# cisco/openh264

Measured on AMD Instinct MI355X. Metric: 1080p frames/sec/GPU at QP=24 CBP; encoder_binary_comparison SHA1 pass, higher is better.
Workload: dtype u8

## Files before the change

### openh264_amd/csrc/kernels/inter_mb.h

```cpp
#pragma once
#include "frame_kernels.h"
#include "../common/gom_rc.h"


#if defined(WH_EMU)
#include <stdio.h>
static long g_wh_win_stat[40];
static void wh_win_stat_dump() {
  if (!getenv ("WELSHIP_WIN_STATS")) return;
  fprintf (stderr, "welship mb stat: skip %ld bg/static %ld intra %ld p16x16 %ld p16x8 %ld p8x16 %ld p8x8 %ld renamed-skip %ld | searches 16x16 %ld 16x8/8x16 %ld 8x8 %ld, diamond steps %ld %ld %ld | refinements %ld %ld %ld | skip tests %ld with transform %ld\n",
           g_wh_win_stat[8], g_wh_win_stat[9], g_wh_win_stat[10], g_wh_win_stat[11], g_wh_win_stat[12], g_wh_win_stat[13], g_wh_win_stat[14], g_wh_win_stat[15], g_wh_win_stat[16], g_wh_win_stat[17], g_wh_win_stat[18],
           g_wh_win_stat[19], g_wh_win_stat[20], g_wh_win_stat[21], g_wh_win_stat[22], g_wh_win_stat[23], g_wh_win_stat[24], g_wh_win_stat[25], g_wh_win_stat[26]);
  fprintf (stderr, "welship window stat: P macroblocks %ld, reloads %ld, adopted %ld, first loads %ld, mid-walk reloads %ld, chroma predictions inside the window %ld / from the picture %ld\n", g_wh_win_stat[0], g_wh_win_stat[1], g_wh_win_stat[2], g_wh_win_stat[3], g_wh_win_stat[4], g_wh_win_stat[5], g_wh_win_stat[6]);
}
struct WhWinStatInit { WhWinStatInit() { atexit (wh_win_stat_dump); } };
static WhWinStatInit g_wh_win_stat_init;
#define WH_STAT_WIN(i) (++g_wh_win_stat[i])
#define WH_STAT_BLK(base, bw, bh) (++g_wh_win_stat[(base) + ((bw) == 16 && (bh) == 16 ? 0 : (bw) == 8 && (bh) == 8 ? 2 : 1)])
#else
#define WH_STAT_WIN(i) ((void)0)
#define WH_STAT_BLK(base, bw, bh) ((void)0)
#endif

#define WH_REF_NOT_AVAIL (-2)
#define WH_REF_NOT_IN_LIST (-1)
#define WH_WIN_STRIDE 80
#ifndef WH_WIN_ROWS
#define WH_WIN_ROWS 38
#endif
#define WH_WIN_MARGIN_X 19
#ifndef WH_WIN_MARGIN_Y
#define WH_WIN_MARGIN_Y 11
#endif
#ifndef WH_WIN_START
// ... 339 lines not shown
}

WH_FN void wh_slot_geom (int slot, int* bx, int* by, int* bw, int* bh) {
  if (slot == 0) { *bx = 0; *by = 0; *bw = 16; *bh = 16; }
  else if (slot < WH_SLOT_16x8) { const int i = slot - WH_SLOT_8x8; *bx = (i & 1) * 8; *by = (i >> 1) * 8; *bw = 8; *bh = 8; }
  else if (slot < WH_SLOT_8x16) { const int i = slot - WH_SLOT_16x8; *bx = 0; *by = i * 8; *bw = 16; *bh = 8; }
  else { const int i = slot - WH_SLOT_8x16; *bx = i * 8; *by = 0; *bw = 8; *bh = 16; }
}
WH_FN void wh_slot_pred (const WhMvCache& K, int slot, int* mx, int* my) {
  if (slot == 0) wh_pred_mv (K, 0, 0, 4, 0, mx, my);
  else if (slot < WH_SLOT_16x8) { const int i = slot - WH_SLOT_8x8; wh_pred_mv (K, (i & 1) * 2, (i >> 1) * 2, 2, 0, mx, my); }
  else if (slot < WH_SLOT_8x16) wh_pred_16x8 (K, slot - WH_SLOT_16x8, 0, mx, my);
  else wh_pred_8x16 (K, slot - WH_SLOT_8x16, 0, mx, my);
}

typedef struct WhMe {
  int bx, by, bw, bh;
  int mvpx, mvpy;
  int sad_pred;
  int mvx, mvy;
  int sad_cost, satd_cost;
  int satd_raw;
} WhMe;

typedef struct WhMeCtx {
  int mbx, mby, lambda, use_satd;
  int minx, miny, maxx, maxy;
} WhMeCtx;

WH_FN int wh_cand_sad (const WhInterLds& S, const WhSeqParams& P, const WhPicJob& J, const WhWin& W, const WhMeCtx& C, const WhMe& me, int imx, int imy) {
  const int px = C.mbx * 16 + me.bx + imx, py = C.mby * 16 + me.by + imy;
  if (wh_win_covers (W, px, py, px + me.bw + 3, py + me.bh))
    return wh_sad_win (S, W, me.bx, me.by, me.bw, me.bh, (py - W.y0) * WH_WIN_STRIDE + px - W.x0);
  return wh_sad_global (S, P, J, me.bx, me.by, me.bw, me.bh, px, py);
}

typedef struct WhSccMe {
  const WH_G WhSccJob* job;
  int method;
  uint32_t thr;
  int dir_on, dmx, dmy;
  uint32_t chain;
  uint32_t fme_down;
} WhSccMe;

WH_FN void wh_line_search (const WhInterLds& S, const WhSeqParams& P, const WhPicJob& J, WhWin& W, const WhMeCtx& C, const WhMe& me, bool vertical, int* best, int* bmx, int* bmy) {
  const int lo = vertical ? C.miny : C.minx, hi = vertical ? C.maxy : C.maxx;
  const int px = C.mbx * 16 + me.bx, py = C.mby * 16 + me.by;
  const WH_G uint8_t* ref = (const WH_G uint8_t*)J.ref[0];
// ... 70 lines not shown
    }
    if (stop) break;
  }
  *best = b;
}

WH_FN void wh_me_satd (WhInterLds& S, const WhWin& W, const WhMeCtx& C, WhMe& me, int bmx, int bmy) {
  const int wo = (C.mby * 16 + me.by + bmy - W.y0) * WH_WIN_STRIDE + C.mbx * 16 + me.bx + bmx - W.x0;
  const int nq = (me.bw >> 2) * (me.bh >> 2) * 4;
  WV_SATD_ROWS (me.satd_raw, lane, lane < nq,
                wh_enc4 (S, me.bx + (lane < nq ? wh_tl_col (lane, me.bw) : 0), me.by + (lane < nq ? wh_tl_row (lane, me.bw) : 0)),
                wh_ld4u (W.b->win, wo + (lane < nq ? wh_tl_row (lane, me.bw) * WH_WIN_STRIDE + wh_tl_col (lane, me.bw) : 0)));
  me.satd_cost = me.satd_raw + wh_mvd_cost (C.lambda, me.mvx - me.mvpx, me.mvy - me.mvpy);
}

WH_FN void wh_motion_search (WhInterLds& S, const WhSeqParams& P, const WhPicJob& J, WhWin& W, const WhMeCtx& C, WhMe& me, const WvLaneArr& mvcl, int n_mvc, WhSccMe* Z = nullptr) {
  int bmx = wh_clip3 ((2 + me.mvpx) >> 2, C.minx, C.maxx), bmy = wh_clip3 ((2 + me.mvpy) >> 2, C.miny, C.maxy);
  int best = wh_cand_sad (S, P, J, W, C, me, bmx, bmy) + wh_mvd_cost (C.lambda, bmx * 4 - me.mvpx, bmy * 4 - me.mvpy);
  for (int i = 0; i < n_mvc; ++i) {
    const int cand = WV_LGET (mvcl, i);
    const int cx = wh_clip3 ((2 + wh_mvx (cand)) >> 2, C.minx, C.maxx), cy = wh_clip3 ((2 + wh_mvy (cand)) >> 2, C.miny, C.maxy);
    if (cx != bmx || cy != bmy) {
      const int c = wh_cand_sad (S, P, J, W, C, me, cx, cy) + wh_mvd_cost (C.lambda, cx * 4 - me.mvpx, cy * 4 - me.mvpy);
      if (c < best) { best = c; bmx = cx; bmy = cy; }
    }
  }
  if (Z && Z->dir_on && (Z->dmx | Z->dmy) && Z->dmx >= C.minx && Z->dmx < C.maxx && Z->dmy >= C.miny && Z->dmy < C.maxy) {
    const int c = wh_cand_sad (S, P, J, W, C, me, Z->dmx, Z->dmy) + wh_mvd_cost (C.lambda, Z->dmx * 4 - me.mvpx, Z->dmy * 4 - me.mvpy);
    if ((uint32_t)c < Z->chain) { best = c; bmx = Z->dmx; bmy = Z->dmy; WH_STAT (WH_ST_DIR_TAKEN); }
  }
  const bool diamond = !(best < me.sad_pred);
  WH_STAT_BLK (16, me.bw, me.bh);
  const int bpx = C.mbx * 16 + me.bx, bpy = C.mby * 16 + me.by;
  if (diamond || C.use_satd) wh_win_need (S, P, J, W, bpx + bmx, bpy + bmy, me.bw, me.bh, diamond ? WH_WIN_START : 0);
  if (diamond) {
    int dx = bmx * 4 - me.mvpx, dy = bmy * 4 - me.mvpy;
    int wo = (bpy + bmy - W.y0) * WH_WIN_STRIDE + bpx + bmx - W.x0;
    const int n = (me.bw * me.bh) >> 2;
    int budget = wh_win_room (W, bpx + bmx, bpy + bmy, me.bw, me.bh);
    for (int it = 0; it < 16; ++it) {
      const int cmx = (dx + me.mvpx) >> 2, cmy = (dy + me.mvpy) >> 2;
      if (!(cmx >= C.minx && cmx < C.maxx && cmy >= C.miny && cmy < C.maxy)) break;
      if (it >= budget) {
        if (wh_win_room (W, bpx + cmx, bpy + cmy, me.bw, me.bh) < 1) {
          WH_STAT_WIN (4);
          wh_win_need (S, P, J, W, bpx + cmx, bpy + cmy, me.bw, me.bh, WH_WIN_START);
          wo = (bpy + cmy - W.y0) * WH_WIN_STRIDE + bpx + cmx - W.x0;
        }
        budget = it + wh_max (1, wh_win_room (W, bpx + cmx, bpy + cmy, me.bw, me.bh));
      }
#if defined(WH_EMU)
      if (wh_win_room (W, bpx + cmx, bpy + cmy, me.bw, me.bh) < 1 || wo != (bpy + cmy - W.y0) * WH_WIN_STRIDE + bpx + cmx - W.x0) { fprintf (stderr, "emu: diamond step outside the search window\n"); abort(); }
#endif
      WH_STAT_BLK (19, me.bw, me.bh);
      int pud, plr;
      WV_SUM2 (pud, plr, lane,
               (lane < n ? ([&] () { const int r = wh_sl_row (lane, me.bw), c = wh_sl_col (lane, me.bw);
                                     const uint32_t e = wh_enc4 (S, me.bx + c, me.by + r); const int o = wo + r * WH_WIN_STRIDE + c;
                                     return wh_sad4 (e, wh_ld4u (W.b->win, o - WH_WIN_STRIDE)) | (wh_sad4 (e, wh_ld4u (W.b->win, o + WH_WIN_STRIDE)) << 16); }) () : 0),
               (lane < n ? ([&] () { const int r = wh_sl_row (lane, me.bw), c = wh_sl_col (lane, me.bw);
                                     const uint32_t e = wh_enc4 (S, me.bx + c, me.by + r); const int o = wo + r * WH_WIN_STRIDE + c;
                                     return wh_sad4 (e, wh_ld4u (W.b->win, o - 1)) | (wh_sad4 (e, wh_ld4u (W.b->win, o + 1)) << 16); }) () : 0));
      const int c0 = (pud & 0xffff) + wh_mvd_cost (C.lambda, dx, dy - 4);
      const int c1 = (int) ((unsigned)pud >> 16) + wh_mvd_cost (C.lambda, dx, dy + 4);
      const int c2 = (plr & 0xffff) + wh_mvd_cost (C.lambda, dx - 4, dy);
      const int c3 = (int) ((unsigned)plr >> 16) + wh_mvd_cost (C.lambda, dx + 4, dy);
      const int in_cost = best;
      int ix = 0, iy = 0;
      if (c0 < best) { best = c0; ix = 0; iy = 1; }
      if (c1 < best) { best = c1; ix = 0; iy = -1; }
      if (c2 < best) { best = c2; ix = 1; iy = 0; }
      if (c3 < best) { best = c3; ix = -1; iy = 0; }
      if (best == in_cost) break;
      dx -= ix * 4; dy -= iy * 4;
      wo -= ix + iy * WH_WIN_STRIDE;
    }
    bmx = (dx + me.mvpx) >> 2; bmy = (dy + me.mvpy) >> 2;
    if (Z && Z->method >= 1) {
      if ((uint32_t)best >= Z->thr) {
        WH_STAT (WH_ST_CROSS_V);
        wh_line_search (S, P, J, W, C, me, true, &best, &bmx, &bmy);
        if ((uint32_t)best >= Z->thr) { WH_STAT (WH_ST_CROSS_H); wh_line_search (S, P, J, W, C, me, false, &best, &bmx, &bmy); }
      }
      if (Z->method == 2 && (uint32_t)best >= Z->thr) {
        const int before = best;
        WH_STAT (WH_ST_FME);
        wh_feature_search (S, P, J, Z->job, C, me, Z->thr, &best, &bmx, &bmy);
        if (best < before) WH_STAT (WH_ST_FME_HIT);
        Z->fme_down += (uint32_t) (before - best);
      }
      if (C.use_satd) wh_win_need (S, P, J, W, bpx + bmx, bpy + bmy, me.bw, me.bh, 0);
    }
// ... 274 lines not shown
  const WhMbState* Tm = (avail & WH_AV_TOP) ? (const WhMbState*)&S.nb[36] : nullptr;
  const WhMbState* TRm = (avail & WH_AV_TOPRIGHT) ? (const WhMbState*)&S.nb[72] : nullptr;
  const WhMbState* Lm = (avail & WH_AV_LEFT) ? (const WhMbState*)&S.nb[108] : nullptr;
  const WhMbState* Co = (const WhMbState*)&S.nb[144];
  const int tl_type = TLm ? TLm->mb_type : WH_MB_NONE, t_type = Tm ? Tm->mb_type : WH_MB_NONE;
  const int tr_type = TRm ? TRm->mb_type : WH_MB_NONE, l_type = Lm ? Lm->mb_type : WH_MB_NONE;
  const bool l_inter = WH_IS_INTER (l_type), t_inter = WH_IS_INTER (t_type), tl_inter = WH_IS_INTER (tl_type), tr_inter = WH_IS_INTER (tr_type);
  WhMvCache K;
  WhMeTab T;
  WvLaneArr mvcl;
#if defined(WH_EMU)
  memset (&K, 0, sizeof (K)); memset (&T, 0, sizeof (T)); memset (&mvcl, 0, sizeof (mvcl));
#else
  K.mv = 0; K.ref = 0; T.mv = 0; T.sad = 0; T.satd = 0; T.raw = 0; mvcl = 0;
#endif
#define WH_CACHE_REF(lane) ([&] () { const int r = (lane) / 6, c = (lane) % 6; \
    if (r == 0 && c == 0) return tl_inter ? (int)TLm->ref_idx[3] : TLm ? WH_REF_NOT_IN_LIST : WH_REF_NOT_AVAIL; \
    if (r == 0 && c == 5) return tr_inter ? (int)TRm->ref_idx[2] : TRm ? WH_REF_NOT_IN_LIST : WH_REF_NOT_AVAIL; \
    if (r == 0) return t_inter ? (int)Tm->ref_idx[2 + ((c - 1) >> 1)] : Tm ? WH_REF_NOT_IN_LIST : WH_REF_NOT_AVAIL; \
    if (c == 0) return l_inter ? (int)Lm->ref_idx[((r - 1) >> 1) * 2 + 1] : Lm ? WH_REF_NOT_IN_LIST : WH_REF_NOT_AVAIL; \
    return WH_REF_NOT_AVAIL; }) ()
#define WH_CACHE_MV(lane) ([&] () { const int r = (lane) / 6, c = (lane) % 6; \
    if (r == 0 && c == 0) return tl_inter ? wh_pk_mv (TLm->mv[15][0], TLm->mv[15][1]) : 0; \
    if (r == 0 && c == 5) return tr_inter ? wh_pk_mv (TRm->mv[12][0], TRm->mv[12][1]) : 0; \
    if (r == 0) return t_inter ? wh_pk_mv (Tm->mv[12 + c - 1][0], Tm->mv[12 + c - 1][1]) : 0; \
    if (c == 0) return l_inter ? wh_pk_mv (Lm->mv[(r - 1) * 4 + 3][0], Lm->mv[(r - 1) * 4 + 3][1]) : 0; \
    return 0; }) ()
  WV_LSET_IF (K.ref, lane, lane < 30, WH_CACHE_REF (lane));
  WV_LSET_IF (K.mv, lane, lane < 30, WH_CACHE_MV (lane));
  if (ctl.cell12_valid) {
// ... 66 lines not shown
  int skx = 0, sky = 0;
  bool done = false;

  auto predict_sad_skip = [&] () {
    const int rb = WV_LGET (K.ref, 1), ra = WV_LGET (K.ref, 6);
    int rc = WV_LGET (K.ref, 5);
    const int sb = sadsk1, sa = sadsk3;
    int sc = sadsk2, skip_c = tr_skc;
    if (rc == WH_REF_NOT_AVAIL) { rc = WV_LGET (K.ref, 0); sc = sadsk0; skip_c = tl_skc; }
    if (rb == WH_REF_NOT_AVAIL && rc == WH_REF_NOT_AVAIL && ra != WH_REF_NOT_AVAIL) return sa;
    const int cnt = ((0 == ra) && l_skc) | (((0 == rb) && t_skc) << 1) | (((0 == rc) && skip_c) << 2);
    return cnt == 1 ? sa : cnt == 2 ? sb : cnt == 4 ? sc : wh_median3 (sa, sb, sc);
  };
  const bool try_skip = l_sk || t_sk || tl_sk || tr_sk;
  bool keep_skip = l_sk && t_sk && tr_sk;
  bool b_skip = false;
  const int stale_cbp = ctl.stale_cbp;
  bool bg_coded = false, bg_skip = false, collocated = false;

  if (bgd) {
    keep_skip = keep_skip && !bg_l && !bg_t && !bg_tr;
    const int ref_type_raw = (int)Co->ref_type - 1;
    const bool ref_intra = Co->ref_type != 0 && Co->ref_type != WH_REFTYPE_BACKGROUND && WH_IS_INTRA (ref_type_raw);
    const int ref_qp = Co->ref_qp;
    if (bg_cur && !ref_intra && (ref_qp - qp <= 3  || ref_qp <= 26)) {
      wh_mc_chroma_to (S, P, J, W, mbx, mby, 0, 0, 8, 8, 0, 0, M.pred_c);
      int cb, cr;
      WV_SUM2 (cb, cr, lane, (lane < 16 ? wh_sad4 (* (const uint32_t*)&M.enc_c[lane * 4], * (const uint32_t*)&M.pred_c[lane * 4]) : 0),
               (lane >= 16 && lane < 32 ? wh_sad4 (* (const uint32_t*)&M.enc_c[lane * 4], * (const uint32_t*)&M.pred_c[lane * 4]) : 0));
      const bool too_large = cb > 640 || cr > 640;
      const int chroma_sad = cb + cr, pred_skip = predict_sad_skip();
// ... 101 lines not shown
        done = true;
      }
    }
  }

  if (!done && ((ref_is_p && ref_mb_type == WH_MB_PSKIP) || try_skip)) {
    const int sad_pred_skip = predict_sad_skip();
    wh_pred_skip_mv (K, &skx, &sky);
    const int nx = (mbx << 4) + (skx >> 2), ny = (mby << 4) + (sky >> 2);
    if (!(nx < -29 || nx > (P.mb_w << 4) + 12 || ny < -29 || ny > (P.mb_h << 4) + 12)) {
      wh_mc_luma_to (S, P, J, W, mbx, mby, 0, 0, 16, 16, skx, sky, M.pred_y);
      WH_PROF_SUB (P, M, 4);
      wh_mc_chroma_to (S, P, J, W, mbx, mby, 0, 0, 8, 8, skx, sky, M.pred_c);
      WH_PROF_SUB (P, M, 5);
      int sad_l, sad_c;
      WV_SUM2 (sad_l, sad_c, lane, wh_sad4 (* (const uint32_t*)&S.m.enc_y[lane * 4], * (const uint32_t*)&M.pred_y[lane * 4]),
               (lane < 32 ? wh_sad4 (* (const uint32_t*)&S.m.enc_c[lane * 4], * (const uint32_t*)&M.pred_c[lane * 4]) : 0));
      const int sad_mb = sad_l + sad_c;
      bool ok = sad_mb == 0 || sad_mb < sad_pred_skip || (ref_is_p && ref_mb_type == WH_MB_PSKIP && !ref_mb_bg && sad_mb < Co->skip_sad);
      WH_PROF_SUB (P, M, 6);
      WH_STAT_WIN (25);
      if (!ok) {
        WH_STAT_WIN (26);
        wh_dct_luma16 (M);
        if (wh_try_py_skip (M, qp)) {
          wh_dct_chroma (M);
          if (wh_try_puv_skip (M, qpc)) ok = true;
        }
      }
      if (ok) {
        b_skip = true;
        if (md_using_sad) cost_luma = sad_l;
        else WV_SATD_ROWS (cost_luma, lane, true, wh_enc4 (S, wh_tl_col (lane, 16), wh_tl_row (lane, 16)), * (const uint32_t*)&M.pred_y[wh_tl_row (lane, 16) * 16 + wh_tl_col (lane, 16)]);
        sad_cost0 = md_using_sad ? sad_l : ((HOSTIN && J.sad_cost0) ? (int)S.sad_cost0_in : Co->sad_cost[0]);
        cost_skip_mb = sad_mb;
        p16x = skx; p16y = sky;
      }
    }
// ... 19 lines not shown
    int nm = 1;
    const bool c_l = Lm != nullptr, c_t = Tm != nullptr, c_r = ref_is_p && mbx < P.mb_w - 1, c_b = ref_is_p && mby < P.mb_h - 1;
    const int i_l = 1, i_t = i_l + (c_l ? 1 : 0), i_r = i_t + (c_t ? 1 : 0), i_b = i_r + (c_r ? 1 : 0);
    nm = i_b + (c_b ? 1 : 0);
    WV_LSET (mvcl, 0, il_mv);
    if (c_l) WV_LSET (mvcl, i_l, wh_pk_mv (Lm->p16mv[0], Lm->p16mv[1]));
    if (c_t) WV_LSET (mvcl, i_t, wh_pk_mv (Tm->p16mv[0], Tm->p16mv[1]));
    const int msh = HOSTIN ? J.mvc_shift : 0;
    if (c_r) WV_LSET (mvcl, i_r, wh_pk_mv (S.co_mv[0][0] >> msh, S.co_mv[0][1] >> msh));
    if (c_b) WV_LSET (mvcl, i_b, wh_pk_mv (S.co_mv[1][0] >> msh, S.co_mv[1][1] >> msh));
    me16.sad_pred = sad_pred;
    if (SCC) {
      WhSccMe z;
      z.job = Z; z.method = 1; z.thr = Z->thr16; z.dir_on = 0; z.dmx = 0; z.dmy = 0; z.chain = 0; z.fme_down = 0;
      wh_motion_search (S, P, J, W, C, me16, mvcl, nm, &z);
    } else wh_motion_search (S, P, J, W, C, me16, mvcl, nm);
    p16x = me16.mvx; p16y = me16.mvy;
    cost_luma = me16.satd_cost;
    mb_type = WH_MB_P16x16;
    sad_pred16 = sad_pred;
  }

  WH_PROF_MARK (P, M, 2);
  bool intra = false;
  WhIntraResult ir;
  if (!done && il_intra) {
    if (b_skip && cost_luma <= i16c.best_cost) { mb_type = WH_MB_PSKIP; done = true; }
    else { (void)wh_intra_md_enc_p<LOW ? 0 : -1, XWG> (M, P, J, mbx, mby, avail, qp, qpc, 0x7fffffff, &ir, &i16c, stale_cbp); intra = true; done = true; }
  }
  if (!done) {
    if (wh_intra_md_enc_p<LOW ? 0 : -1, XWG> (M, P, J, mbx, mby, avail, qp, qpc, cost_luma, &ir, &i16c, stale_cbp)) { intra = true; done = true; }
  }
  if (!done && b_skip) { mb_type = WH_MB_PSKIP; done = true; }
  WH_PROF_MARK (P, M, 3);
  auto publish_guess = [&] (int fin) {
    if (X.last_mv) {
      WV_LANES_BEGIN (lane)
      if (lane == 0) *X.last_mv = fin;
      WV_LANES_END
    }
  };
  const bool searched = !done;
  if (done && !intra) publish_guess (mb_type == WH_MB_PSKIP ? wh_pk_mv (skx, sky) : wh_pk_mv (p16x, p16y));

  if (searched) {
    wh_me_store (T, WH_SLOT_16x16, me16);
    WV_LSET (mvcl, 0, il_mv);
    int order0 = -1, order1 = -1, order2 = -1;
    bool chain = false;
    bool merged = false;
    if (SCC) {
      const int32_t* v8 = (const int32_t*)G.cold_pv;
      const int s8_0 = v8[0], s8_1 = v8[1], s8_2 = v8[2], s8_3 = v8[3];
      const int avg = (s8_0 + s8_1 + s8_2 + s8_3) >> 2;
      const int d0 = (s8_0 >> 6) - (avg >> 6), d1 = (s8_1 >> 6) - (avg >> 6), d2 = (s8_2 >> 6) - (avg >> 6), d3 = (s8_3 >> 6) - (avg >> 6);
      if (d0 * d0 + d1 * d1 + d2 * d2 + d3 * d3 >= 20) {
// ... 73 lines not shown
      else if (sign != 15) { order0 = 0; order1 = 1; order2 = 2; chain = true; }
    } else {
      order0 = 0; order1 = 1; order2 = 2; chain = true;
    }
    int best_cost = cost_luma;
    for (int oi = 0; oi < 3; ++oi) {
      const int g = oi == 0 ? order0 : oi == 1 ? order1 : order2;
      if (g < 0) break;
      const int first = g == 0 ? WH_SLOT_8x8 : g == 1 ? WH_SLOT_16x8 : WH_SLOT_8x16, cnt = g == 0 ? 4 : 2;
      int c = 0;
      for (int i = 0; i < cnt; ++i) {
        WhMe m;
        wh_slot_geom (first + i, &m.bx, &m.by, &m.bw, &m.bh);
        m.sad_pred = g == 0 ? sad_pred16 >> 2 : sad_pred16 >> 1;
        wh_slot_pred (K, first + i, &m.mvpx, &m.mvpy);
        wh_motion_search (S, P, J, W, C, m, mvcl, 1);
        wh_cache_set (K, m.bx >> 2, m.by >> 2, m.bw >> 2, m.bh >> 2, 0, m.mvx, m.mvy);
        wh_me_store (T, first + i, m);
        c += m.satd_cost;
      }
      if (oi == 0) {
        if (c < best_cost) { best_cost = c; mb_type = g == 0 ? WH_MB_P8x8 : g == 1 ? WH_MB_P16x8 : WH_MB_P8x16; }
        else if (chain) break;
      } else if (c <= best_cost) { best_cost = c; mb_type = g == 1 ? WH_MB_P16x8 : WH_MB_P8x16; }
    }

    WH_PROF_MARK (P, M, 4);
    const int satd_in_md = use_satd;
    int best_sad = 0, best_satd = 0;
    if (mb_type == WH_MB_P8x8) {
      WV_LSET (K.ref, 9, WH_REF_NOT_AVAIL); WV_LSET (K.ref, 21, WH_REF_NOT_AVAIL);
// ... 6 lines not shown
        wh_slot_geom (first + i, &m.bx, &m.by, &m.bw, &m.bh);
        wh_me_fetch (T, first + i, m);
        wh_slot_pred (K, first + i, &m.mvpx, &m.mvpy);
        wh_refine_frac (S, P, J, W, C, m, satd_in_md, merged ? 1 : 0);
        wh_cache_set (K, m.bx >> 2, m.by >> 2, m.bw >> 2, m.bh >> 2, 0, m.mvx, m.mvy);
        {
          const int bx4 = m.bx >> 2, by4 = m.by >> 2, w4 = m.bw >> 2, h4 = m.bh >> 2;
          WV_LANES_BEGIN (lane)
          if (lane < w4 * h4) {
            const int r = (by4 + (w4 == 4 ? lane >> 2 : lane >> 1)) * 4 + bx4 + (lane & (w4 - 1));
            S.mv_out[r][0] = (int16_t)m.mvx; S.mv_out[r][1] = (int16_t)m.mvy; S.mvp_out[r][0] = (int16_t)m.mvpx; S.mvp_out[r][1] = (int16_t)m.mvpy;
          }
          WV_LANES_END
        }
        best_sad += m.sad_cost; best_satd += m.satd_cost;
        wh_mc_chroma_to (S, P, J, W, mbx, mby, m.bx >> 1, m.by >> 1, m.bw >> 1, m.bh >> 1, m.mvx, m.mvy, M.pred_c);
        if (mb_type == WH_MB_P16x16) { me16.mvx = m.mvx; me16.mvy = m.mvy; }
      }
    }
    if (mb_type == WH_MB_P16x16) {
      int sl, sc;
      WV_SUM2 (sl, sc, lane, wh_sad4 (* (const uint32_t*)&M.enc_y[lane * 4], * (const uint32_t*)&M.pred_y[lane * 4]),
               (lane < 32 ? wh_sad4 (* (const uint32_t*)&M.enc_c[lane * 4], * (const uint32_t*)&M.pred_c[lane * 4]) : 0));
      cost_skip_mb = sl + sc;
    }
    sad_cost0 = best_sad;
    cost_luma = md_using_sad ? best_sad : best_satd;

    WH_PROF_MARK (P, M, 5);
    publish_guess (wh_pk_mv (p16x, p16y));
  }
  if (searched) {
    wh_dct_luma16 (M);
    cbp = wh_enc_inter_y (M, qp);
    const int cbp_c = wh_encrec_chroma (M, qpc, 0);
    cbp |= cbp_c << 4;
    wh_idct_luma16 (M);
    wh_idct_chroma (M);
    if (mb_type == WH_MB_P16x16 && cbp == 0) {
      int sx, sy;
      wh_pred_skip_mv (K, &sx, &sy);
      if (sx == me16.mvx && sy == me16.mvy) { mb_type = WH_MB_PSKIP; skx = sx; sky = sy; }
    }
  }

  WH_PROF_MARK (P, M, 6);
  const bool is_skip = mb_type == WH_MB_PSKIP;
  WH_STAT_WIN (intra ? 10 : (bg_coded || scd_coded) ? 9 : (is_skip && b_skip) ? 8 : is_skip ? 15 : mb_type == WH_MB_P16x16 ? 11 : mb_type == WH_MB_P16x8 ? 12 : mb_type == WH_MB_P8x16 ? 13 : 14);
  WH_G WhMbState* Ms = (WH_G WhMbState*)J.mbs + xy;
  WH_G WhMbRecord* Rs = (WH_G WhMbRecord*)J.records + xy;
  if (intra) {
    WV_LANES_BEGIN (lane)
    if (lane < 16) { wh_st_x<XWG> ((WH_G uint32_t*)&Ms->mv[lane][0], 0u); Rs->mvd[lane][0] = 0; Rs->mvd[lane][1] = 0; }
    if (lane < 2) Rs->mv_tr[lane] = 0;
    if (lane < 4) { wh_st_x<XWG> (&Ms->ref_idx[lane], (int8_t)-1); Rs->ref_idx[lane] = -1; Rs->sub_type[lane] = 0; }
    if (lane == 0) { wh_st_x<XWG> (&Ms->sad_cost[0], 0); wh_st_x<XWG> ((WH_G uint32_t*)&Ms->p16mv[0], (uint32_t)wh_pk_mv (p16x, p16y)); wh_st_x<XWG> (&Ms->skip_sad, 0); if (HOSTIN && J.sad_cost0) (J.sad_cost0_out ? (WH_G int32_t*)J.sad_cost0_out : (WH_G int32_t*)J.sad_cost0)[xy] = 0; }
    WV_LANES_END
// ... 113 lines not shown
```

### openh264_amd/csrc/kernels/wave.h

```cpp
#pragma once
#include <stdint.h>

#if defined(WH_EMU)
#define WH_FN static inline
#define WH_HDFN static inline
#define WH_CONST static const
#if defined(WH_EMU_REVERSE)
#define WV_LANES_BEGIN(lane) for (int lane = 63; lane >= 0; --lane) {
#else
#define WV_LANES_BEGIN(lane) for (int lane = 0; lane < 64; ++lane) {
#endif
#define WV_LANES_END }
#define WH_UNIFORM_VALUE(x) ((void)0)
#define WV_SYNC() ((void)0)
#define WV_GLOBAL_FENCE() ((void)0)
#define WV_SUM(dst, lane, expr)                                   \
  do { int _s = 0; for (int lane = 0; lane < 64; ++lane) _s += (int)(expr); (dst) = _s; } while (0)
#define WV_ARGMIN(dst_key, dst_lane, lane, valid, key)            \
  do { int _bk = 0x7fffffff, _bl = -1;                            \
       for (int lane = 0; lane < 64; ++lane) if (valid) { int _k = (int)(key); if (_k < _bk) { _bk = _k; _bl = lane; } } \
       (dst_key) = _bk; (dst_lane) = _bl; } while (0)
#define WV_ANY(dst, lane, expr)                                   \
  do { int _a = 0; for (int lane = 0; lane < 64; ++lane) _a |= ((expr) ? 1 : 0); (dst) = _a; } while (0)
#define WV_SUM2(dst_a, dst_b, lane, expr_a, expr_b)               \
  do { int _sa = 0, _sb = 0; for (int lane = 0; lane < 64; ++lane) { _sa += (int)(expr_a); _sb += (int)(expr_b); } (dst_a) = _sa; (dst_b) = _sb; } while (0)
#define WV_QUADSUM_TAB(tab, lane, expr)                           \
  do { int _t[64]; for (int lane = 0; lane < 64; ++lane) _t[lane] = (int)(expr); \
       for (int _q = 0; _q < 16; ++_q) { const int _s = _t[4 * _q] + _t[4 * _q + 1] + _t[4 * _q + 2] + _t[4 * _q + 3]; \
         for (int _k = 0; _k < 4; ++_k) (tab).v[4 * _q + _k] = _s; } } while (0)
#define WV_PAIRSUM_TAB(tab, lane, expr)                           \
  do { int _t[64]; for (int lane = 0; lane < 64; ++lane) _t[lane] = (int)(expr); \
       for (int _p = 0; _p < 32; ++_p) { (tab).v[2 * _p] = (tab).v[2 * _p + 1] = _t[2 * _p] + _t[2 * _p + 1]; } } while (0)
#define WV_LSHUF(dst, src, lane, idx)                             \
  do { WvLaneArr _s = (src); for (int lane = 0; lane < 64; ++lane) (dst).v[lane] = _s.v[(idx) & 63]; } while (0)
#define WV_QUADSUM4(d0, d1, d2, d3, lane, expr)                   \
  do { int _q[4] = {0, 0, 0, 0}; for (int lane = 0; lane < 16; ++lane) _q[lane >> 2] += (int)(expr); \
       (d0) = _q[0]; (d1) = _q[1]; (d2) = _q[2]; (d3) = _q[3]; } while (0)
#define WV_ROWSUM4(d0, d1, d2, d3, lane, expr)                    \
  do { int _q[4] = {0, 0, 0, 0}; for (int lane = 0; lane < 64; ++lane) _q[lane >> 4] += (int)(expr); \
       (d0) = _q[0]; (d1) = _q[1]; (d2) = _q[2]; (d3) = _q[3]; } while (0)
// ... 89 lines not shown
#define WV_ARGMIN(dst_key, dst_lane, lane, valid, key)            \
  do { const int lane = (int)(threadIdx.x & 63);                  \
       const bool _ok = (valid);                                  \
       int _k = _ok ? (int)(key) : 0x7fffffff;                    \
       const int _m = wh_wave_min_i32 (_k);                       \
       const unsigned long long _b = __ballot (_ok && _k == _m);  \
       (dst_key) = _m; (dst_lane) = _b ? (int)__builtin_ctzll (_b) : -1; } while (0)
#define WV_ANY(dst, lane, expr)                                   \
  do { const int lane = (int)(threadIdx.x & 63); (dst) = __ballot ((expr)) != 0ULL; } while (0)
#define WV_SUM2(dst_a, dst_b, lane, expr_a, expr_b)               \
  do { const int lane = wh_lane_id(); int _va = (int)(expr_a), _vb = (int)(expr_b); \
       _va += WH_DPP (_va, 0xB1); _vb += WH_DPP (_vb, 0xB1); _va += WH_DPP (_va, 0x4E); _vb += WH_DPP (_vb, 0x4E); \
       _va += WH_DPP (_va, 0x141); _vb += WH_DPP (_vb, 0x141); _va += WH_DPP (_va, 0x140); _vb += WH_DPP (_vb, 0x140); \
       _va += WH_DPP_ROWS (_va, 0x142, 0xA); _vb += WH_DPP_ROWS (_vb, 0x142, 0xA); _va += WH_DPP_ROWS (_va, 0x143, 0xC); _vb += WH_DPP_ROWS (_vb, 0x143, 0xC); \
       (dst_a) = __builtin_amdgcn_readlane (_va, 63); (dst_b) = __builtin_amdgcn_readlane (_vb, 63); } while (0)
#define WV_QUADSUM_TAB(tab, lane, expr)                           \
  do { const int lane = wh_lane_id(); int _v = (int)(expr);       \
       _v += WH_DPP (_v, 0xB1); _v += WH_DPP (_v, 0x4E); (tab) = _v; } while (0)
#define WV_PAIRSUM_TAB(tab, lane, expr)                           \
  do { const int lane = wh_lane_id(); int _v = (int)(expr);       \
       _v += WH_DPP (_v, 0xB1); (tab) = _v; } while (0)
#define WV_LSHUF(dst, src, lane, idx)                             \
  do { const int lane = wh_lane_id(); (dst) = __builtin_amdgcn_ds_bpermute ((int)(idx) << 2, (src)); } while (0)
#define WV_QUADSUM4(d0, d1, d2, d3, lane, expr)                   \
  do { const int lane = wh_lane_id(); int _v = (int)(expr);       \
       _v += WH_DPP (_v, 0xB1); _v += WH_DPP (_v, 0x4E);          \
       (d0) = __builtin_amdgcn_readlane (_v, 0); (d1) = __builtin_amdgcn_readlane (_v, 4); (d2) = __builtin_amdgcn_readlane (_v, 8); (d3) = __builtin_amdgcn_readlane (_v, 12); } while (0)
#define WV_ROWSUM4(d0, d1, d2, d3, lane, expr)                    \
  do { const int lane = wh_lane_id(); int _v = (int)(expr);       \
       _v += WH_DPP (_v, 0xB1); _v += WH_DPP (_v, 0x4E); _v += WH_DPP (_v, 0x141); _v += WH_DPP (_v, 0x140); \
// ... 137 lines not shown
```

Measured before the change: 27490.

## Memoize per-quadrant SADs from 16x16 search to serve partition searches and skip reuse

Adds a per-macroblock SAD memo held in wave lanes. The 16x16 candidate and diamond evaluations record quadrant SADs keyed by integer MV, so the 16x8, 8x16 and 8x8 partition searches can look up candidate and diamond SADs instead of recomputing them, and only load the search window when the memo misses. It also moves the P16x16 skip-cost computation to the point where a skip decision is actually made. It reuses the skip test's chroma prediction and luma DCT when the final vector equals the skip vector. The cost is extra DPP reductions, lane lookups and memo bookkeeping, plus more complex window-loading logic.

```diff
diff --git a/openh264_amd/csrc/kernels/inter_mb.h b/openh264_amd/csrc/kernels/inter_mb.h
--- a/openh264_amd/csrc/kernels/inter_mb.h
+++ b/openh264_amd/csrc/kernels/inter_mb.h
@@ -11,13 +11,18 @@
   fprintf (stderr, "welship mb stat: skip %ld bg/static %ld intra %ld p16x16 %ld p16x8 %ld p8x16 %ld p8x8 %ld renamed-skip %ld | searches 16x16 %ld 16x8/8x16 %ld 8x8 %ld, diamond steps %ld %ld %ld | refinements %ld %ld %ld | skip tests %ld with transform %ld\n",
            g_wh_win_stat[8], g_wh_win_stat[9], g_wh_win_stat[10], g_wh_win_stat[11], g_wh_win_stat[12], g_wh_win_stat[13], g_wh_win_stat[14], g_wh_win_stat[15], g_wh_win_stat[16], g_wh_win_stat[17], g_wh_win_stat[18],
            g_wh_win_stat[19], g_wh_win_stat[20], g_wh_win_stat[21], g_wh_win_stat[22], g_wh_win_stat[23], g_wh_win_stat[24], g_wh_win_stat[25], g_wh_win_stat[26]);
+  fprintf (stderr, "welship sad memo stat: partition single SADs %ld served %ld, partition diamond steps %ld served %ld, most entries %ld, integer skip vectors %ld, final vector equals skip vector %ld\n",
+           g_wh_win_stat[27], g_wh_win_stat[28], g_wh_win_stat[29], g_wh_win_stat[30], g_wh_win_stat[31], g_wh_win_stat[32], g_wh_win_stat[33]);
   fprintf (stderr, "welship window stat: P macroblocks %ld, reloads %ld, adopted %ld, first loads %ld, mid-walk reloads %ld, chroma predictions inside the window %ld / from the picture %ld\n", g_wh_win_stat[0], g_wh_win_stat[1], g_wh_win_stat[2], g_wh_win_stat[3], g_wh_win_stat[4], g_wh_win_stat[5], g_wh_win_stat[6]);
 }
 struct WhWinStatInit { WhWinStatInit() { atexit (wh_win_stat_dump); } };
 static WhWinStatInit g_wh_win_stat_init;
 #define WH_STAT_WIN(i) (++g_wh_win_stat[i])
 #define WH_STAT_BLK(base, bw, bh) (++g_wh_win_stat[(base) + ((bw) == 16 && (bh) == 16 ? 0 : (bw) == 8 && (bh) == 8 ? 2 : 1)])
+#define WH_STAT_MAX(i, v) do { if ((long)(v) > g_wh_win_stat[i]) g_wh_win_stat[i] = (long)(v); } while (0)
+extern "C" int welship_emu_win_stats (long* out, int n) { for (int i = 0; i < n && i < 40; ++i) out[i] = g_wh_win_stat[i]; return 40; }
 #else
+#define WH_STAT_MAX(i, v) ((void)0)
 #define WH_STAT_WIN(i) ((void)0)
 #define WH_STAT_BLK(base, bw, bh) ((void)0)
 #endif
@@ -387,6 +392,70 @@
   else wh_pred_8x16 (K, slot - WH_SLOT_8x16, 0, mx, my);
 }
 
+#ifndef WH_SAD_MEMO
+#define WH_SAD_MEMO 1
+#endif
+#ifndef WH_SKIP_COST_LATE
+#define WH_SKIP_COST_LATE 1
+#endif
+#ifndef WH_SKIP_REUSE
+#define WH_SKIP_REUSE 1
+#endif
+#define WH_MEMO_CAP 64
+#define WH_MEMO_NOKEY ((int)0x80008000u)
+typedef struct WhSadMemo { WvLaneArr key, up, lo; int n; } WhSadMemo;
+WH_FN void wh_memo_clear (WhSadMemo& Q) {
+#if defined(WH_EMU)
+  memset (&Q.up, 0, sizeof (Q.up)); memset (&Q.lo, 0, sizeof (Q.lo));
+  for (int i = 0; i < 64; ++i) Q.key.v[i] = WH_MEMO_NOKEY;
+#else
+  Q.key = WH_MEMO_NOKEY; Q.up = 0; Q.lo = 0;
+#endif
+  Q.n = 0;
+}
+WH_FN void wh_memo_put (WhSadMemo& Q, int imx, int imy, int up, int lo) {
+  if (Q.n < WH_MEMO_CAP) {
+    WV_LSET (Q.key, Q.n, wh_pk_mv (imx, imy)); WV_LSET (Q.up, Q.n, up); WV_LSET (Q.lo, Q.n, lo);
+    ++Q.n;
+    WH_STAT_MAX (31, Q.n);
+  }
+}
+WH_FN int wh_memo_blk (int up, int lo, int bx, int by, int bw, int bh) {
+  const int q0 = up & 0xffff, q1 = (int) ((unsigned)up >> 16), q2 = lo & 0xffff, q3 = (int) ((unsigned)lo >> 16);
+  if (bw == 16) return bh == 16 ? q0 + q1 + q2 + q3 : by ? q2 + q3 : q0 + q1;
+  if (bh == 16) return bx ? q1 + q3 : q0 + q2;
+  return by ? (bx ? q3 : q2) : (bx ? q1 : q0);
+}
+WH_FN bool wh_memo_get (const WhSadMemo& Q, int imx, int imy, int bx, int by, int bw, int bh, int* sad) {
+  int l;
+  WV_LFIND (l, Q.key, wh_pk_mv (imx, imy));
+  if (l < 0) return false;
+  *sad = wh_memo_blk (WV_LGET (Q.up, l), WV_LGET (Q.lo, l), bx, by, bw, bh);
+  return true;
+}
+WH_FN void wh_sad_win_q (const WhInterLds& S, const WhWin& W, int wo, int* up, int* lo) {
+  int u, l;
+  WV_SUMQ (u, l, lane, wh_sad4 (wh_enc4 (S, (lane & 3) * 4, lane >> 2), wh_ld4u (W.b->win, wo + (lane >> 2) * WH_WIN_STRIDE + (lane & 3) * 4)));
+  *up = u; *lo = l;
+}
+WH_FN void wh_sad_global_q (const WhInterLds& S, const WhSeqParams& P, const WhPicJob& J, int px, int py, int* up, int* lo) {
+  int u, l;
+  const WH_G uint8_t* ref = (const WH_G uint8_t*)J.ref[0];
+  WV_SUMQ (u, l, lane, ([&] () { const WH_G uint8_t* t = ref + (ptrdiff_t) (py + (lane >> 2)) * P.rec_stride_y + px + (lane & 3) * 4;
+                                  return wh_sad4 (wh_enc4 (S, (lane & 3) * 4, lane >> 2), wh_pack4 (t[0], t[1], t[2], t[3])); }) ());
+  *up = u; *lo = l;
+}
+#if defined(WH_EMU)
+extern "C" void welship_emu_quadrant_sums (const uint8_t* e, const uint8_t* r, int* out) {
+#define WH_T_SAD(k) wh_sad4 (* (const uint32_t*)&e[lane * 4], * (const uint32_t*)&r[256 * (k) + lane * 4])
+  WV_SUMQ (out[0], out[1], lane, WH_T_SAD (0));
+  WV_SUM (out[2], lane, WH_T_SAD (0));
+  WV_SUM2Q (out[3], out[4], out[5], out[6], out[7], out[8], out[9], out[10], lane, WH_T_SAD (0) | (WH_T_SAD (1) << 16), WH_T_SAD (2) | (WH_T_SAD (3) << 16));
+  WV_SUM2 (out[11], out[12], lane, WH_T_SAD (0) | (WH_T_SAD (1) << 16), WH_T_SAD (2) | (WH_T_SAD (3) << 16));
+#undef WH_T_SAD
+}
+#endif
+
 typedef struct WhMe {
   int bx, by, bw, bh;
   int mvpx, mvpy;
@@ -406,6 +475,20 @@
   if (wh_win_covers (W, px, py, px + me.bw + 3, py + me.bh))
     return wh_sad_win (S, W, me.bx, me.by, me.bw, me.bh, (py - W.y0) * WH_WIN_STRIDE + px - W.x0);
   return wh_sad_global (S, P, J, me.bx, me.by, me.bw, me.bh, px, py);
+}
+WH_FN int wh_cand_sad_memo (const WhInterLds& S, const WhSeqParams& P, const WhPicJob& J, const WhWin& W, const WhMeCtx& C, const WhMe& me, int imx, int imy, WhSadMemo* Q) {
+  if (!Q) return wh_cand_sad (S, P, J, W, C, me, imx, imy);
+  const bool whole = me.bw == 16 && me.bh == 16;
+  int sad;
+  if (!whole) WH_STAT_WIN (27);
+  if (wh_memo_get (*Q, imx, imy, me.bx, me.by, me.bw, me.bh, &sad)) { if (!whole) WH_STAT_WIN (28); return sad; }
+  if (!whole) return wh_cand_sad (S, P, J, W, C, me, imx, imy);
+  const int px = C.mbx * 16 + imx, py = C.mby * 16 + imy;
+  int up, lo;
+  if (wh_win_covers (W, px, py, px + 16 + 3, py + 16)) wh_sad_win_q (S, W, (py - W.y0) * WH_WIN_STRIDE + px - W.x0, &up, &lo);
+  else wh_sad_global_q (S, P, J, px, py, &up, &lo);
+  wh_memo_put (*Q, imx, imy, up, lo);
+  return wh_memo_blk (up, lo, 0, 0, 16, 16);
 }
 
 typedef struct WhSccMe {
@@ -506,14 +589,15 @@
   me.satd_cost = me.satd_raw + wh_mvd_cost (C.lambda, me.mvx - me.mvpx, me.mvy - me.mvpy);
 }
 
-WH_FN void wh_motion_search (WhInterLds& S, const WhSeqParams& P, const WhPicJob& J, WhWin& W, const WhMeCtx& C, WhMe& me, const WvLaneArr& mvcl, int n_mvc, WhSccMe* Z = nullptr) {
+WH_FN void wh_motion_search (WhInterLds& S, const WhSeqParams& P, const WhPicJob& J, WhWin& W, const WhMeCtx& C, WhMe& me, const WvLaneArr& mvcl, int n_mvc, WhSccMe* Z = nullptr, WhSadMemo* Q = nullptr) {
+  const bool whole = me.bw == 16 && me.bh == 16, served = Q && !whole;
   int bmx = wh_clip3 ((2 + me.mvpx) >> 2, C.minx, C.maxx), bmy = wh_clip3 ((2 + me.mvpy) >> 2, C.miny, C.maxy);
-  int best = wh_cand_sad (S, P, J, W, C, me, bmx, bmy) + wh_mvd_cost (C.lambda, bmx * 4 - me.mvpx, bmy * 4 - me.mvpy);
+  int best = wh_cand_sad_memo (S, P, J, W, C, me, bmx, bmy, Q) + wh_mvd_cost (C.lambda, bmx * 4 - me.mvpx, bmy * 4 - me.mvpy);
   for (int i = 0; i < n_mvc; ++i) {
     const int cand = WV_LGET (mvcl, i);
     const int cx = wh_clip3 ((2 + wh_mvx (cand)) >> 2, C.minx, C.maxx), cy = wh_clip3 ((2 + wh_mvy (cand)) >> 2, C.miny, C.maxy);
     if (cx != bmx || cy != bmy) {
-      const int c = wh_cand_sad (S, P, J, W, C, me, cx, cy) + wh_mvd_cost (C.lambda, cx * 4 - me.mvpx, cy * 4 - me.mvpy);
+      const int c = wh_cand_sad_memo (S, P, J, W, C, me, cx, cy, Q) + wh_mvd_cost (C.lambda, cx * 4 - me.mvpx, cy * 4 - me.mvpy);
       if (c < best) { best = c; bmx = cx; bmy = cy; }
     }
   }
@@ -524,39 +608,71 @@
   const bool diamond = !(best < me.sad_pred);
   WH_STAT_BLK (16, me.bw, me.bh);
   const int bpx = C.mbx * 16 + me.bx, bpy = C.mby * 16 + me.by;
-  if (diamond || C.use_satd) wh_win_need (S, P, J, W, bpx + bmx, bpy + bmy, me.bw, me.bh, diamond ? WH_WIN_START : 0);
+  bool win_set = !served;
+  if (win_set ? (diamond || C.use_satd) : (!diamond && C.use_satd)) wh_win_need (S, P, J, W, bpx + bmx, bpy + bmy, me.bw, me.bh, diamond ? WH_WIN_START : 0);
   if (diamond) {
     int dx = bmx * 4 - me.mvpx, dy = bmy * 4 - me.mvpy;
     int wo = (bpy + bmy - W.y0) * WH_WIN_STRIDE + bpx + bmx - W.x0;
     const int n = (me.bw * me.bh) >> 2;
-    int budget = wh_win_room (W, bpx + bmx, bpy + bmy, me.bw, me.bh);
+    int budget = win_set ? wh_win_room (W, bpx + bmx, bpy + bmy, me.bw, me.bh) : 0;
     for (int it = 0; it < 16; ++it) {
       const int cmx = (dx + me.mvpx) >> 2, cmy = (dy + me.mvpy) >> 2;
       if (!(cmx >= C.minx && cmx < C.maxx && cmy >= C.miny && cmy < C.maxy)) break;
-      if (it >= budget) {
-        if (wh_win_room (W, bpx + cmx, bpy + cmy, me.bw, me.bh) < 1) {
-          WH_STAT_WIN (4);
+      WH_STAT_BLK (19, me.bw, me.bh);
+      int s0 = 0, s1 = 0, s2 = 0, s3 = 0;
+      bool hit = false;
+      if (served) {
+        WH_STAT_WIN (29);
+        hit = wh_memo_get (*Q, cmx, cmy - 1, me.bx, me.by, me.bw, me.bh, &s0) && wh_memo_get (*Q, cmx, cmy + 1, me.bx, me.by, me.bw, me.bh, &s1) &&
+              wh_memo_get (*Q, cmx - 1, cmy, me.bx, me.by, me.bw, me.bh, &s2) && wh_memo_get (*Q, cmx + 1, cmy, me.bx, me.by, me.bw, me.bh, &s3);
+        if (hit) WH_STAT_WIN (30);
+      }
+      if (!hit) {
+        if (!win_set) {
           wh_win_need (S, P, J, W, bpx + cmx, bpy + cmy, me.bw, me.bh, WH_WIN_START);
           wo = (bpy + cmy - W.y0) * WH_WIN_STRIDE + bpx + cmx - W.x0;
+          budget = it + wh_max (1, wh_win_room (W, bpx + cmx, bpy + cmy, me.bw, me.bh));
+          win_set = true;
+        } else if (it >= budget) {
+          if (wh_win_room (W, bpx + cmx, bpy + cmy, me.bw, me.bh) < 1) {
+            WH_STAT_WIN (4);
+            wh_win_need (S, P, J, W, bpx + cmx, bpy + cmy, me.bw, me.bh, WH_WIN_START);
+            wo = (bpy + cmy - W.y0) * WH_WIN_STRIDE + bpx + cmx - W.x0;
+          }
+          budget = it + wh_max (1, wh_win_room (W, bpx + cmx, bpy + cmy, me.bw, me.bh));
         }
-        budget = it + wh_max (1, wh_win_room (W, bpx + cmx, bpy + cmy, me.bw, me.bh));
-      }
 #if defined(WH_EMU)
-      if (wh_win_room (W, bpx + cmx, bpy + cmy, me.bw, me.bh) < 1 || wo != (bpy + cmy - W.y0) * WH_WIN_STRIDE + bpx + cmx - W.x0) { fprintf (stderr, "emu: diamond step outside the search window\n"); abort(); }
-#endif
-      WH_STAT_BLK (19, me.bw, me.bh);
-      int pud, plr;
-      WV_SUM2 (pud, plr, lane,
-               (lane < n ? ([&] () { const int r = wh_sl_row (lane, me.bw), c = wh_sl_col (lane, me.bw);
-                                     const uint32_t e = wh_enc4 (S, me.bx + c, me.by + r); const int o = wo + r * WH_WIN_STRIDE + c;
-                                     return wh_sad4 (e, wh_ld4u (W.b->win, o - WH_WIN_STRIDE)) | (wh_sad4 (e, wh_ld4u (W.b->win, o + WH_WIN_STRIDE)) << 16); }) () : 0),
-               (lane < n ? ([&] () { const int r = wh_sl_row (lane, me.bw), c = wh_sl_col (lane, me.bw);
-                                     const uint32_t e = wh_enc4 (S, me.bx + c, me.by + r); const int o = wo + r * WH_WIN_STRIDE + c;
-                                     return wh_sad4 (e, wh_ld4u (W.b->win, o - 1)) | (wh_sad4 (e, wh_ld4u (W.b->win, o + 1)) << 16); }) () : 0));
-      const int c0 = (pud & 0xffff) + wh_mvd_cost (C.lambda, dx, dy - 4);
-      const int c1 = (int) ((unsigned)pud >> 16) + wh_mvd_cost (C.lambda, dx, dy + 4);
-      const int c2 = (plr & 0xffff) + wh_mvd_cost (C.lambda, dx - 4, dy);
-      const int c3 = (int) ((unsigned)plr >> 16) + wh_mvd_cost (C.lambda, dx + 4, dy);
+        if (wh_win_room (W, bpx + cmx, bpy + cmy, me.bw, me.bh) < 1 || wo != (bpy + cmy - W.y0) * WH_WIN_STRIDE + bpx + cmx - W.x0) { fprintf (stderr, "emu: diamond step outside the search window\n"); abort(); }
+#endif
+        int pud, plr;
+        if (Q && whole) {
+          int a0, a1, a2, a3, b0, b1, b2, b3;
+          WV_SUM2Q (a0, a1, a2, a3, b0, b1, b2, b3, lane,
+                    ([&] () { const int r = lane >> 2, c = (lane & 3) * 4;
+                              const uint32_t e = wh_enc4 (S, c, r); const int o = wo + r * WH_WIN_STRIDE + c;
+                              return wh_sad4 (e, wh_ld4u (W.b->win, o - WH_WIN_STRIDE)) | (wh_sad4 (e, wh_ld4u (W.b->win, o + WH_WIN_STRIDE)) << 16); }) (),
+                    ([&] () { const int r = lane >> 2, c = (lane & 3) * 4;
+                              const uint32_t e = wh_enc4 (S, c, r); const int o = wo + r * WH_WIN_STRIDE + c;
+                              return wh_sad4 (e, wh_ld4u (W.b->win, o - 1)) | (wh_sad4 (e, wh_ld4u (W.b->win, o + 1)) << 16); }) ());
+          wh_memo_put (*Q, cmx, cmy - 1, (int) (((unsigned)a0 & 0xffffu) | ((unsigned)a1 << 16)), (int) (((unsigned)a2 & 0xffffu) | ((unsigned)a3 << 16)));
+          wh_memo_put (*Q, cmx, cmy + 1, (int) (((unsigned)a0 >> 16) | ((unsigned)a1 & 0xffff0000u)), (int) (((unsigned)a2 >> 16) | ((unsigned)a3 & 0xffff0000u)));
+          wh_memo_put (*Q, cmx - 1, cmy, (int) (((unsigned)b0 & 0xffffu) | ((unsigned)b1 << 16)), (int) (((unsigned)b2 & 0xffffu) | ((unsigned)b3 << 16)));
+          wh_memo_put (*Q, cmx + 1, cmy, (int) (((unsigned)b0 >> 16) | ((unsigned)b1 & 0xffff0000u)), (int) (((unsigned)b2 >> 16) | ((unsigned)b3 & 0xffff0000u)));
+          pud = a0 + a1 + a2 + a3; plr = b0 + b1 + b2 + b3;
+        } else
+        WV_SUM2 (pud, plr, lane,
+                 (lane < n ? ([&] () { const int r = wh_sl_row (lane, me.bw), c = wh_sl_col (lane, me.bw);
+                                       const uint32_t e = wh_enc4 (S, me.bx + c, me.by + r); const int o = wo + r * WH_WIN_STRIDE + c;
+                                       return wh_sad4 (e, wh_ld4u (W.b->win, o - WH_WIN_STRIDE)) | (wh_sad4 (e, wh_ld4u (W.b->win, o + WH_WIN_STRIDE)) << 16); }) () : 0),
+                 (lane < n ? ([&] () { const int r = wh_sl_row (lane, me.bw), c = wh_sl_col (lane, me.bw);
+                                       const uint32_t e = wh_enc4 (S, me.bx + c, me.by + r); const int o = wo + r * WH_WIN_STRIDE + c;
+                                       return wh_sad4 (e, wh_ld4u (W.b->win, o - 1)) | (wh_sad4 (e, wh_ld4u (W.b->win, o + 1)) << 16); }) () : 0));
+        s0 = pud & 0xffff; s1 = (int) ((unsigned)pud >> 16); s2 = plr & 0xffff; s3 = (int) ((unsigned)plr >> 16);
+      }
+      const int c0 = s0 + wh_mvd_cost (C.lambda, dx, dy - 4);
+      const int c1 = s1 + wh_mvd_cost (C.lambda, dx, dy + 4);
+      const int c2 = s2 + wh_mvd_cost (C.lambda, dx - 4, dy);
+      const int c3 = s3 + wh_mvd_cost (C.lambda, dx + 4, dy);
       const int in_cost = best;
       int ix = 0, iy = 0;
       if (c0 < best) { best = c0; ix = 0; iy = 1; }
@@ -568,6 +684,7 @@
       wo -= ix + iy * WH_WIN_STRIDE;
     }
     bmx = (dx + me.mvpx) >> 2; bmy = (dy + me.mvpy) >> 2;
+    if (served && C.use_satd) wh_win_need (S, P, J, W, bpx + bmx, bpy + bmy, me.bw, me.bh, 0);
     if (Z && Z->method >= 1) {
       if ((uint32_t)best >= Z->thr) {
         WH_STAT (WH_ST_CROSS_V);
@@ -872,6 +989,9 @@
 #else
   K.mv = 0; K.ref = 0; T.mv = 0; T.sad = 0; T.satd = 0; T.raw = 0; mvcl = 0;
 #endif
+  WhSadMemo Q;
+  wh_memo_clear (Q);
+  constexpr bool MEMO = WH_SAD_MEMO && !SCC;
 #define WH_CACHE_REF(lane) ([&] () { const int r = (lane) / 6, c = (lane) % 6; \
     if (r == 0 && c == 0) return tl_inter ? (int)TLm->ref_idx[3] : TLm ? WH_REF_NOT_IN_LIST : WH_REF_NOT_AVAIL; \
     if (r == 0 && c == 5) return tr_inter ? (int)TRm->ref_idx[2] : TRm ? WH_REF_NOT_IN_LIST : WH_REF_NOT_AVAIL; \
@@ -968,7 +1088,7 @@
   };
   const bool try_skip = l_sk || t_sk || tl_sk || tr_sk;
   bool keep_skip = l_sk && t_sk && tr_sk;
-  bool b_skip = false;
+  bool b_skip = false, skip_tested = false;
   const int stale_cbp = ctl.stale_cbp;
   bool bg_coded = false, bg_skip = false, collocated = false;
 
@@ -1100,6 +1220,14 @@
       wh_mc_chroma_to (S, P, J, W, mbx, mby, 0, 0, 8, 8, skx, sky, M.pred_c);
       WH_PROF_SUB (P, M, 5);
       int sad_l, sad_c;
+      if (MEMO && ((skx | sky) & 3) == 0) {
+        int up, lo;
+        WH_STAT_WIN (32);
+        WV_SUMQ (up, lo, lane, wh_sad4 (* (const uint32_t*)&S.m.enc_y[lane * 4], * (const uint32_t*)&M.pred_y[lane * 4]));
+        WV_SUM (sad_c, lane, (lane < 32 ? wh_sad4 (* (const uint32_t*)&S.m.enc_c[lane * 4], * (const uint32_t*)&M.pred_c[lane * 4]) : 0));
+        wh_memo_put (Q, skx >> 2, sky >> 2, up, lo);
+        sad_l = wh_memo_blk (up, lo, 0, 0, 16, 16);
+      } else
       WV_SUM2 (sad_l, sad_c, lane, wh_sad4 (* (const uint32_t*)&S.m.enc_y[lane * 4], * (const uint32_t*)&M.pred_y[lane * 4]),
                (lane < 32 ? wh_sad4 (* (const uint32_t*)&S.m.enc_c[lane * 4], * (const uint32_t*)&M.pred_c[lane * 4]) : 0));
       const int sad_mb = sad_l + sad_c;
@@ -1108,6 +1236,7 @@
       WH_STAT_WIN (25);
       if (!ok) {
         WH_STAT_WIN (26);
+        skip_tested = true;
         wh_dct_luma16 (M);
         if (wh_try_py_skip (M, qp)) {
           wh_dct_chroma (M);
@@ -1157,7 +1286,7 @@
       WhSccMe z;
       z.job = Z; z.method = 1; z.thr = Z->thr16; z.dir_on = 0; z.dmx = 0; z.dmy = 0; z.chain = 0; z.fme_down = 0;
       wh_motion_search (S, P, J, W, C, me16, mvcl, nm, &z);
-    } else wh_motion_search (S, P, J, W, C, me16, mvcl, nm);
+    } else wh_motion_search (S, P, J, W, C, me16, mvcl, nm, nullptr, MEMO ? &Q : nullptr);
     p16x = me16.mvx; p16y = me16.mvy;
     cost_luma = me16.satd_cost;
     mb_type = WH_MB_P16x16;
@@ -1183,6 +1312,13 @@
       WV_LANES_END
     }
   };
+  auto cost_skip_p16 = [&] () {
+    int sl, sc;
+    WV_SUM2 (sl, sc, lane, wh_sad4 (* (const uint32_t*)&M.enc_y[lane * 4], * (const uint32_t*)&M.pred_y[lane * 4]),
+             (lane < 32 ? wh_sad4 (* (const uint32_t*)&M.enc_c[lane * 4], * (const uint32_t*)&M.pred_c[lane * 4]) : 0));
+    return sl + sc;
+  };
+  bool skip_kept = false;
   const bool searched = !done;
   if (done && !intra) publish_guess (mb_type == WH_MB_PSKIP ? wh_pk_mv (skx, sky) : wh_pk_mv (p16x, p16y));
 
@@ -1286,7 +1422,7 @@
         wh_slot_geom (first + i, &m.bx, &m.by, &m.bw, &m.bh);
         m.sad_pred = g == 0 ? sad_pred16 >> 2 : sad_pred16 >> 1;
         wh_slot_pred (K, first + i, &m.mvpx, &m.mvpy);
-        wh_motion_search (S, P, J, W, C, m, mvcl, 1);
+        wh_motion_search (S, P, J, W, C, m, mvcl, 1, nullptr, MEMO ? &Q : nullptr);
         wh_cache_set (K, m.bx >> 2, m.by >> 2, m.bw >> 2, m.bh >> 2, 0, m.mvx, m.mvy);
         wh_me_store (T, first + i, m);
         c += m.satd_cost;
@@ -1323,16 +1459,12 @@
           WV_LANES_END
         }
         best_sad += m.sad_cost; best_satd += m.satd_cost;
-        wh_mc_chroma_to (S, P, J, W, mbx, mby, m.bx >> 1, m.by >> 1, m.bw >> 1, m.bh >> 1, m.mvx, m.mvy, M.pred_c);
+        if (mb_type == WH_MB_P16x16 && skip_tested && m.mvx == skx && m.mvy == sky) { skip_kept = WH_SKIP_REUSE && !SCC; WH_STAT_WIN (33); }
+        if (!skip_kept) wh_mc_chroma_to (S, P, J, W, mbx, mby, m.bx >> 1, m.by >> 1, m.bw >> 1, m.bh >> 1, m.mvx, m.mvy, M.pred_c);
         if (mb_type == WH_MB_P16x16) { me16.mvx = m.mvx; me16.mvy = m.mvy; }
       }
     }
-    if (mb_type == WH_MB_P16x16) {
-      int sl, sc;
-      WV_SUM2 (sl, sc, lane, wh_sad4 (* (const uint32_t*)&M.enc_y[lane * 4], * (const uint32_t*)&M.pred_y[lane * 4]),
-               (lane < 32 ? wh_sad4 (* (const uint32_t*)&M.enc_c[lane * 4], * (const uint32_t*)&M.pred_c[lane * 4]) : 0));
-      cost_skip_mb = sl + sc;
-    }
+    if (!WH_SKIP_COST_LATE && mb_type == WH_MB_P16x16) cost_skip_mb = cost_skip_p16();
     sad_cost0 = best_sad;
     cost_luma = md_using_sad ? best_sad : best_satd;
 
@@ -1340,7 +1472,7 @@
     publish_guess (wh_pk_mv (p16x, p16y));
   }
   if (searched) {
-    wh_dct_luma16 (M);
+    if (!skip_kept) wh_dct_luma16 (M);
     cbp = wh_enc_inter_y (M, qp);
     const int cbp_c = wh_encrec_chroma (M, qpc, 0);
     cbp |= cbp_c << 4;
@@ -1349,7 +1481,7 @@
     if (mb_type == WH_MB_P16x16 && cbp == 0) {
       int sx, sy;
       wh_pred_skip_mv (K, &sx, &sy);
-      if (sx == me16.mvx && sy == me16.mvy) { mb_type = WH_MB_PSKIP; skx = sx; sky = sy; }
+      if (sx == me16.mvx && sy == me16.mvy) { mb_type = WH_MB_PSKIP; skx = sx; sky = sy; if (WH_SKIP_COST_LATE) cost_skip_mb = cost_skip_p16(); }
     }
   }
 
diff --git a/openh264_amd/csrc/kernels/wave.h b/openh264_amd/csrc/kernels/wave.h
--- a/openh264_amd/csrc/kernels/wave.h
+++ b/openh264_amd/csrc/kernels/wave.h
@@ -24,6 +24,15 @@
   do { int _a = 0; for (int lane = 0; lane < 64; ++lane) _a |= ((expr) ? 1 : 0); (dst) = _a; } while (0)
 #define WV_SUM2(dst_a, dst_b, lane, expr_a, expr_b)               \
   do { int _sa = 0, _sb = 0; for (int lane = 0; lane < 64; ++lane) { _sa += (int)(expr_a); _sb += (int)(expr_b); } (dst_a) = _sa; (dst_b) = _sb; } while (0)
+#define WV_SUMQ(dst_up, dst_lo, lane, expr)                       \
+  do { int _q[4] = {0, 0, 0, 0}; for (int lane = 0; lane < 64; ++lane) _q[((lane >> 5) << 1) | ((lane >> 1) & 1)] += (int)(expr); \
+       (dst_up) = (int) ((unsigned)_q[0] | ((unsigned)_q[1] << 16)); (dst_lo) = (int) ((unsigned)_q[2] | ((unsigned)_q[3] << 16)); } while (0)
+#define WV_SUM2Q(a0, a1, a2, a3, b0, b1, b2, b3, lane, expr_a, expr_b) \
+  do { int _qa[4] = {0, 0, 0, 0}, _qb[4] = {0, 0, 0, 0};          \
+       for (int lane = 0; lane < 64; ++lane) { const int _q = ((lane >> 5) << 1) | ((lane >> 1) & 1); _qa[_q] += (int)(expr_a); _qb[_q] += (int)(expr_b); } \
+       (a0) = _qa[0]; (a1) = _qa[1]; (a2) = _qa[2]; (a3) = _qa[3]; (b0) = _qb[0]; (b1) = _qb[1]; (b2) = _qb[2]; (b3) = _qb[3]; } while (0)
+#define WV_LFIND(dst_lane, tab, val)                              \
+  do { int _l = -1; for (int _i = 63; _i >= 0; --_i) if ((tab).v[_i] == (val)) _l = _i; (dst_lane) = _l; } while (0)
 #define WV_QUADSUM_TAB(tab, lane, expr)                           \
   do { int _t[64]; for (int lane = 0; lane < 64; ++lane) _t[lane] = (int)(expr); \
        for (int _q = 0; _q < 16; ++_q) { const int _s = _t[4 * _q] + _t[4 * _q + 1] + _t[4 * _q + 2] + _t[4 * _q + 3]; \
@@ -143,6 +152,21 @@
        _va += WH_DPP (_va, 0x141); _vb += WH_DPP (_vb, 0x141); _va += WH_DPP (_va, 0x140); _vb += WH_DPP (_vb, 0x140); \
        _va += WH_DPP_ROWS (_va, 0x142, 0xA); _vb += WH_DPP_ROWS (_vb, 0x142, 0xA); _va += WH_DPP_ROWS (_va, 0x143, 0xC); _vb += WH_DPP_ROWS (_vb, 0x143, 0xC); \
        (dst_a) = __builtin_amdgcn_readlane (_va, 63); (dst_b) = __builtin_amdgcn_readlane (_vb, 63); } while (0)
+#define WV_SUMQ(dst_up, dst_lo, lane, expr)                       \
+  do { const int lane = wh_lane_id(); int _v = (int)(expr);       \
+       _v += WH_DPP (_v, 0xB1); _v = (int) ((unsigned)_v << 16) + WH_DPP (_v, 0x4E); \
+       _v += WH_DPP (_v, 0x124); _v += WH_DPP (_v, 0x128);         \
+       _v += WH_DPP_ROWS (_v, 0x142, 0xA);                        \
+       (dst_up) = __builtin_amdgcn_readlane (_v, 31); (dst_lo) = __builtin_amdgcn_readlane (_v, 63); } while (0)
+#define WV_SUM2Q(a0, a1, a2, a3, b0, b1, b2, b3, lane, expr_a, expr_b) \
+  do { const int lane = wh_lane_id(); int _va = (int)(expr_a), _vb = (int)(expr_b); \
+       _va += WH_DPP (_va, 0xB1); _vb += WH_DPP (_vb, 0xB1); _va += WH_DPP (_va, 0x124); _vb += WH_DPP (_vb, 0x124); _va += WH_DPP (_va, 0x128); _vb += WH_DPP (_vb, 0x128); \
+       (a0) = __builtin_amdgcn_readlane (_va, 0) + __builtin_amdgcn_readlane (_va, 16); (a1) = __builtin_amdgcn_readlane (_va, 2) + __builtin_amdgcn_readlane (_va, 18); \
+       (a2) = __builtin_amdgcn_readlane (_va, 32) + __builtin_amdgcn_readlane (_va, 48); (a3) = __builtin_amdgcn_readlane (_va, 34) + __builtin_amdgcn_readlane (_va, 50); \
+       (b0) = __builtin_amdgcn_readlane (_vb, 0) + __builtin_amdgcn_readlane (_vb, 16); (b1) = __builtin_amdgcn_readlane (_vb, 2) + __builtin_amdgcn_readlane (_vb, 18); \
+       (b2) = __builtin_amdgcn_readlane (_vb, 32) + __builtin_amdgcn_readlane (_vb, 48); (b3) = __builtin_amdgcn_readlane (_vb, 34) + __builtin_amdgcn_readlane (_vb, 50); } while (0)
+#define WV_LFIND(dst_lane, tab, val)                              \
+  do { const unsigned long long _b = __ballot ((tab) == (val)); (dst_lane) = _b ? (int)__builtin_ctzll (_b) : -1; } while (0)
 #define WV_QUADSUM_TAB(tab, lane, expr)                           \
   do { const int lane = wh_lane_id(); int _v = (int)(expr);       \
        _v += WH_DPP (_v, 0xB1); _v += WH_DPP (_v, 0x4E); (tab) = _v; } while (0)
```

After: 27010. 1.7% lower.
